# dalek-cryptography/zkp

Measured on AMD Instinct MI355X. Metric: proofs/sec + batch-verifies/sec, CMZ13 10-attr credential, 1/2/4/8 MI355X, higher is better.
Workload: dtype u32x9 (29-bit limbs, u64 accumulate)

## Files before the change

### include/zkp_mi355x.h

```cpp
#ifndef ZKP_MI355X_H
#define ZKP_MI355X_H

#include <stddef.h>
#include <stdint.h>

#ifdef __cplusplus
extern "C" {
#endif

#define ZKP_OK 0
#define ZKP_ERR_HIP (-1)
#define ZKP_ERR_ARG (-2)
#define ZKP_ERR_NO_DEVICE (-3)
#define ZKP_ERR_OOM (-4)

#define ZKP_VARTIME 0
#define ZKP_CT 1

typedef struct zkp_ctx zkp_ctx;

int zkp_ctx_create(zkp_ctx** out, int device_id);
void zkp_ctx_destroy(zkp_ctx* ctx);
int zkp_ctx_set_stream(zkp_ctx* ctx, void* hip_stream);
int zkp_ctx_synchronize(zkp_ctx* ctx);
// ... 285 lines not shown
  ZKP_K_REDUCE = 2,
  ZKP_K_SORT = 3,
  ZKP_K_BUCKET = 4,
  ZKP_K_COMBINE = 5,
  ZKP_K_TRANSCRIPT = 6,
  ZKP_K_SCALARS = 7,
  ZKP_K_TABLES = 8,
  ZKP_K_COUNT = 9
};
int zkp_ctx_last_timing(zkp_ctx* ctx, float* kernel_ms , float* total_ms);
int zkp_ctx_last_kernels(zkp_ctx* ctx, int kind, char* buf, size_t cap);
int zkp_ctx_set_profiling(zkp_ctx* ctx, int enabled);

#ifdef ZKP_BUILD_TEST_HOOKS
int zkp_debug_quad_selftest(zkp_ctx* ctx, uint32_t n, const uint8_t* pairs , uint8_t* out );
int zkp_debug_row_selftest(zkp_ctx* ctx, uint32_t n, const uint8_t* pairs , uint8_t* out );
int zkp_debug_wave_cycles(zkp_ctx* ctx, uint64_t* out, uint32_t cap);
int zkp_debug_sha512(zkp_ctx* ctx, uint64_t n, const uint8_t* msgs, const uint64_t* offsets , uint8_t* out );
int zkp_debug_last_schedule(zkp_ctx* ctx, char* buf, size_t cap);
int zkp_debug_ragged_blocks(const uint8_t* transcripts, uint32_t N, uint32_t* idx, uint32_t* blocks, uint32_t cap);
int zkp_debug_fill_workspace(zkp_ctx* ctx, size_t min_bytes, uint32_t word);
size_t zkp_debug_ws_bytes(zkp_ctx* ctx);
size_t zkp_debug_ws_count(zkp_ctx* ctx, const uint8_t* needle, size_t len);
enum { ZKP_TESTOPT_DUMMY_LAUNCHES = 1001, ZKP_TESTOPT_GENERIC_CLASSIFIER = 1002, ZKP_TESTOPT_WAVE_CYCLES = 1003, ZKP_TESTOPT_PIP_MERGE = 1004, ZKP_TESTOPT_VOUCH_REDUCED = 1005, ZKP_TESTOPT_PIP_RUN_CAP = 1006 };
#endif

#ifdef __cplusplus
}
#endif
#endif
```

### zkp_amd/csrc/hot_tables.h

```cpp
#pragma once
#include "dev_layout.h"
#include "stmt_pairs.h"

namespace zkp {

#ifndef ZKP_HOT_W
#define ZKP_HOT_W 7
#endif
constexpr int HOT_W = ZKP_HOT_W;
constexpr int HOT_WINDOWS = (257 + HOT_W - 1) / HOT_W;
constexpr int HOT_HALF = 1 << (HOT_W - 1);
constexpr int HOT_ROW = HOT_HALF + 1;
constexpr int HOT_SLOTS = 64;
constexpr int HOT_CLASSES = HOT_SLOTS + 3;
constexpr int CLASS_COMB = HOT_SLOTS, CLASS_LADDER = HOT_SLOTS + 1, CLASS_GROUP = HOT_SLOTS + 2;
constexpr uint32_t GROUP_MIN_USES = 10;
constexpr size_t HOT_SLOT_NIELS = (size_t)HOT_WINDOWS * HOT_ROW;
constexpr int HOT_ROW_CHUNKS = HOT_ROW * (int)(sizeof(dev_niels) / 16);
constexpr int HOT_COPIES = 16;
static_assert(HOT_W >= 6 && HOT_W <= 7 && HOT_W * HOT_WINDOWS >= 258, "fixed-base window shape");
constexpr bool HOT_LDS_ROWS = HOT_ROW_CHUNKS <= 256;

constexpr int HOT_FOLD_WINDOWS = 252 / HOT_W;
static_assert(HOT_FOLD_WINDOWS * HOT_W == 252 && HOT_FOLD_WINDOWS < HOT_WINDOWS, "the folded walk ends at bit 252");

constexpr uint32_t hot_pattern_word(int i, int n = HOT_WINDOWS) {
  uint32_t v = 0;
  for (int w = 0; w < n; ++w) {
    const int bit = HOT_W * w + HOT_W - 1;
    if (bit / 32 == i) v |= 1u << (bit % 32);
  }
  return v;
}
__device__ __forceinline__ void hot_recode(uint32_t e[9], const uint32_t s[8], bool fold = false) {
  constexpr uint32_t P[9] = {hot_pattern_word(0), hot_pattern_word(1), hot_pattern_word(2), hot_pattern_word(3), hot_pattern_word(4),
                             hot_pattern_word(5), hot_pattern_word(6), hot_pattern_word(7), hot_pattern_word(8)};
  constexpr uint32_t F[9] = {hot_pattern_word(0, HOT_FOLD_WINDOWS - 1), hot_pattern_word(1, HOT_FOLD_WINDOWS - 1), hot_pattern_word(2, HOT_FOLD_WINDOWS - 1),
                             hot_pattern_word(3, HOT_FOLD_WINDOWS - 1), hot_pattern_word(4, HOT_FOLD_WINDOWS - 1), hot_pattern_word(5, HOT_FOLD_WINDOWS - 1),
                             hot_pattern_word(6, HOT_FOLD_WINDOWS - 1), hot_pattern_word(7, HOT_FOLD_WINDOWS - 1), hot_pattern_word(8, HOT_FOLD_WINDOWS - 1)};
  uint64_t c = 0;
#pragma unroll
  for (int i = 0; i < 8; ++i) {
    c += (uint64_t)s[i] + (fold ? F[i] : P[i]);
    e[i] = (uint32_t)c;
    c >>= 32;
  }
  e[8] = (uint32_t)c + (fold ? F[8] : P[8]);
}
__device__ __forceinline__ void hot_next_digit(uint32_t e[9], uint32_t& mag, uint32_t& neg, bool raw = false) {
  const uint32_t d = e[0] & ((1u << HOT_W) - 1u);
#pragma unroll
  for (int i = 0; i < 8; ++i) e[i] = __builtin_amdgcn_alignbit(e[i + 1], e[i], HOT_W);
  e[8] >>= HOT_W;
  neg = raw ? 0u : (uint32_t)(d < (uint32_t)HOT_HALF);
  mag = raw ? d : neg ? (uint32_t)HOT_HALF - d : d - (uint32_t)HOT_HALF;
}

__global__ void __launch_bounds__(64, 2)
k_hot_bases(uint32_t nh, const dev_affine* __restrict__ pts, dev_ext* __restrict__ bases) {
  const uint32_t h = blockIdx.x * blockDim.x + threadIdx.x;
  if (h >= nh) return;
  ge_p3 b;
  load_affine(b, pts + h);
  ge_pin_vgpr(b);
  store_ext(bases + (size_t)h * HOT_WINDOWS, b);
#pragma unroll 1
  for (int w = 1; w < HOT_WINDOWS; ++w) {
#pragma unroll 1
    for (int k = 0; k < HOT_W - 1; ++k) ge_double<false>(b, b);
    ge_double<true>(b, b);
    store_ext(bases + (size_t)h * HOT_WINDOWS + w, b);
  }
}

__global__ void __launch_bounds__(64, 2)
k_hot_rows(uint32_t nh, const uint32_t* __restrict__ slots, const dev_ext* __restrict__ bases, dev_ext* __restrict__ mult,
           dev_niels* __restrict__ tables) {
  const uint32_t g = blockIdx.x * blockDim.x + threadIdx.x;
  if (g >= nh * HOT_WINDOWS) return;
// ... 326 lines not shown
            wd[4 * i + 0] = (wd[4 * i + 0] & ~m) | (x.x & m); wd[4 * i + 1] = (wd[4 * i + 1] & ~m) | (x.y & m);
            wd[4 * i + 2] = (wd[4 * i + 2] & ~m) | (x.z & m); wd[4 * i + 3] = (wd[4 * i + 3] & ~m) | (x.w & m);
          }
        }
      } else {
        const uint4* ent = rep + (size_t)mag * (sizeof(dev_niels) / 16) * HOT_COPIES + copy;
#pragma unroll
        for (int i = 0; i < 7; ++i) {
          const uint4 x = ent[i * HOT_COPIES];
          wd[4 * i + 0] = x.x; wd[4 * i + 1] = x.y; wd[4 * i + 2] = x.z; wd[4 * i + 3] = x.w;
        }
      }
      ge_niels q;
      fe_set(q.ypx, wd); fe_set(q.ymx, wd + 9); fe_set(q.xy2d, wd + 18);
      ge_niels_cneg(q, neg);
      if (w == 0) ge_from_niels(acc, q);
      else ge_madd(acc, acc, q);
    }
  }
}

__device__ __forceinline__ uint32_t xbar_fetch(int src_lane_x4, uint32_t v) { return (uint32_t)__builtin_amdgcn_ds_bpermute(src_lane_x4, (int)v); }

__device__ __forceinline__ void fixed_base_xbar(ge_p3& acc, uint32_t e[9], const uint4* __restrict__ rows, bool fold = false) {
  const uint32_t lane = threadIdx.x & 63u;
  constexpr int SETS = HOT_HALF / 32;
  static_assert(HOT_HALF == 32 * SETS && SETS >= 1 && SETS <= 2, "the crossbar walk holds sets of 32 entries");
  const uint4* my = rows + (size_t)(1u + (lane & 31u)) * 7u + (lane >> 5) * 4u;
  const uint32_t last = lane < 32u ? 3u : 2u;
  uint4 r[SETS][4];
#pragma unroll
  for (int s = 0; s < SETS; ++s)
#pragma unroll
    for (int q = 0; q < 4; ++q) r[s][q] = my[(size_t)s * 32 * 7 + (q < 3 ? (uint32_t)q : last)];
  const int windows = fold ? HOT_FOLD_WINDOWS : HOT_WINDOWS;
#pragma unroll 1
  for (int w = 0; w < windows; ++w) {
    uint32_t mag, neg;
    hot_next_digit(e, mag, neg, fold && w == HOT_FOLD_WINDOWS - 1);
    const uint32_t nz = (uint32_t)(mag != 0u);
    const uint32_t m1 = mag - nz;
    const int src = (int)((m1 & 31u) << 2);
    uint32_t wd[28];
#pragma unroll
    for (int s = 0; s < SETS; ++s) {
      uint32_t t[28];
#pragma unroll
      for (int q = 0; q < 4; ++q) {
        t[4 * q + 0] = xbar_fetch(src, r[s][q].x); t[4 * q + 1] = xbar_fetch(src, r[s][q].y);
        t[4 * q + 2] = xbar_fetch(src, r[s][q].z); t[4 * q + 3] = xbar_fetch(src, r[s][q].w);
      }
#pragma unroll
      for (int q = 0; q < 3; ++q) {
        t[16 + 4 * q + 0] = xbar_fetch(src + 128, r[s][q].x); t[16 + 4 * q + 1] = xbar_fetch(src + 128, r[s][q].y);
        t[16 + 4 * q + 2] = xbar_fetch(src + 128, r[s][q].z);
        if (q < 2) t[16 + 4 * q + 3] = xbar_fetch(src + 128, r[s][q].w);
      }
      if (s == 0) {
#pragma unroll
        for (int i = 0; i < 27; ++i) wd[i] = t[i];
      } else {
        const bool hi = m1 >= 32u;
#pragma unroll
        for (int i = 0; i < 27; ++i) wd[i] = hi ? t[i] : wd[i];
      }
    }
    if (w + 1 < windows) {
      const uint4* nx = my + (size_t)(w + 1) * HOT_ROW_CHUNKS;
#pragma unroll
      for (int s = 0; s < SETS; ++s)
#pragma unroll
        for (int q = 0; q < 4; ++q) r[s][q] = nx[(size_t)s * 32 * 7 + (q < 3 ? (uint32_t)q : last)];
    }
    const uint32_t m = 0u - nz;
#pragma unroll
    for (int i = 0; i < 27; ++i) wd[i] &= m;
    wd[0] |= nz ^ 1u;
    wd[9] |= nz ^ 1u;
    ge_niels q;
    fe_set(q.ypx, wd); fe_set(q.ymx, wd + 9); fe_set(q.xy2d, wd + 18);
    ge_niels_cneg(q, neg);
    if (w == 0) ge_from_niels(acc, q);
    else ge_madd(acc, acc, q);
  }
}

}
```

### zkp_amd/csrc/zkp_kernels.hip

```cpp
#include <hip/hip_runtime.h>
#include <sys/syscall.h>
#include <unistd.h>
#include <cassert>
#include <cctype>
#include <cstdio>
#include <cstring>
#include <algorithm>
#include <atomic>
#include <functional>
#include <map>
#include <memory>
#include <mutex>
#include <set>
#include <string>
#include <unordered_map>
#include <vector>
#include "../../include/zkp_mi355x.h"
#include "dev_layout.h"

using namespace zkp;

__device__ __forceinline__ uint32_t sel8(const uint32_t w[8], int j) {
  uint32_t r = w[0];
#pragma unroll
// ... 165 lines not shown
    }
    ZKP_WAVE_T1(2);
  } else if (vb < ladder_blocks + comb_blocks + group_blocks) {
    if constexpr (CT && TEETH == 16) {
      if constexpr (LOOKUP == LOOKUP_XBAR)
        comb_group_xbar((vb - ladder_blocks - comb_blocks) * XBAR_BLOCK_TERMS, n_group, list + class_start[CLASS_GROUP], scalars, pidx, slot_of, comb, partial, hot_lds, no_carry != 0);
      else
        comb_group_block((vb - ladder_blocks - comb_blocks) * 256u, n_group, list + class_start[CLASS_GROUP], scalars, pidx, slot_of, comb, partial, hot_lds, no_carry != 0);
    }
    ZKP_WAVE_T1(3);
  } else {
    const uint32_t hb = vb - ladder_blocks - comb_blocks - group_blocks;
    if (hb >= blk_start[HOT_SLOTS]) return;
    uint32_t c = 0;
    while (blk_start[c + 1] <= hb) ++c;
    const uint4* src = reinterpret_cast<const uint4*>(tables + (size_t)c * HOT_SLOT_NIELS);
    const uint32_t i = (hb - blk_start[c]) * 256 + threadIdx.x;
    const bool live = i < class_start[c + 1] - class_start[c];
    const uint32_t t = live ? list[class_start[c] + i] : 0u;
    uint32_t s[8], e[9];
    ge_p3 acc;
    ge_identity(acc);
    if constexpr (LOOKUP == LOOKUP_XBAR) {
      if (hb * 256u + (threadIdx.x & ~63u) - blk_start[c] * 256u >= class_start[c + 1] - class_start[c]) return;
#pragma unroll
      for (int q = 0; q < 8; ++q) s[q] = 0;
      if (live) load_vec<2>(s, scalars + 32 * (size_t)t);
      const bool fold = CT && no_carry;
      uint32_t flip = 0;
      if (fold) flip = sc_fold_sign(s);
      hot_recode(e, s, fold);
      fixed_base_xbar(acc, e, src, fold);
      if (fold) ge_cneg(acc, flip);
    } else {
      if (live) {
        load_vec<2>(s, scalars + 32 * (size_t)t);
        hot_recode(e, s);
      }
      fixed_base_block<LOOKUP == LOOKUP_SCAN>(acc, e, live, src, hot_lds);
    }
    if (live) store_ext(partial + t, acc);
    ZKP_WAVE_T1(4);
  }
}

struct msm_map {
  uint32_t N = 0, nc = 0;
  const uint32_t* order = nullptr;
};
__device__ __forceinline__ uint32_t msm_of_lane(const msm_map& m, uint32_t p) {
  if (!m.order) return p;
  const uint32_t q = p / m.N;
  return (p - q * m.N) * m.nc + m.order[q];
}

// ... 687 lines not shown
#pragma unroll 1
  for (int k = 0; k < shift; ++k) q_double(U, U, q);
  if (level > 0) {
    const dev_ext* ain = A_in + (size_t)w * in_stride + (size_t)m * j;
#pragma unroll 1
    for (int i = 0; i < m; ++i) {
      q_load_ext(t, ain + i, q);
      q_add(U, U, t, q);
    }
  }
  q_store_ext(A_out + (size_t)w * out_stride + j, U, q);
  if (R_out) q_store_ext(R_out + (size_t)w * out_stride + j, run, q);
}
__global__ void __launch_bounds__(256, 2)
k_pip_reduce_lvl(uint32_t n_out, uint32_t total, uint32_t in_stride, uint32_t out_stride, int level, int m, int shift,
                 const dev_ext* __restrict__ A_in, const dev_ext* __restrict__ R_in,
                 dev_ext* __restrict__ A_out, dev_ext* __restrict__ R_out) {
  const uint32_t gt = blockIdx.x * blockDim.x + threadIdx.x;
  const uint32_t g = gt >> 2;
  const int q = (int)(gt & 3u);
  if (g >= total) return;
  pip_reduce_quad(g, q, n_out, in_stride, out_stride, level, m, shift, A_in, R_in, A_out, R_out);
}

__global__ void __launch_bounds__(256)
k_pip_combine(int W1, int C, uint32_t in_stride, int level, int m, int shift, const dev_ext* __restrict__ A_in, const dev_ext* __restrict__ R_in,
              dev_ext* __restrict__ T_all, const uint32_t* __restrict__ invalid, uint8_t* __restrict__ out_point, uint32_t* __restrict__ status,
              uint32_t shared_flags ) {
  const uint32_t b = blockIdx.x;
  dev_ext* T = T_all + (size_t)b * W1;
  const uint32_t g = threadIdx.x >> 2;
  const int q = (int)(threadIdx.x & 3u);
  if (g < (uint32_t)W1) pip_reduce_quad(b * (uint32_t)W1 + g, q, 1u, in_stride, 1u, level, m, shift, A_in, R_in, T_all, nullptr);
  __syncthreads();
  __shared__ uint32_t Tl[64 * 36];
  if (g < (uint32_t)W1) {
    qpt t;
    q_load_ext(t, T + g, q);
    if (g + 1 < (uint32_t)W1) {
      qcached cc;
      q_to_cached(cc, t, q);
      t.c = cc.c;
    }
#pragma unroll
    for (int i = 0; i < 9; ++i) Tl[36 * g + 9 * q + i] = t.c.v[i];
  }
// ... 681 lines not shown
  bool batch_encode_user = false;
  int comb_teeth = 4;
  int ct_single_use_tables = -1;
  struct { bool offered = false, active = false; const tr_op* ops = nullptr; uint32_t n_ops = 0; const uint64_t* tables = nullptr; uint32_t N = 0; tr_bufs bufs{};
           uint8_t* ts = nullptr; uint32_t* saved = nullptr; uint32_t* failed = nullptr; uint32_t tail = 0;
           bool steps = false; tr_steps_dev sd; uint64_t* img = nullptr; } pending_tr;
  int debug_dummy_launches = 0;
  bool stmt_classify = true;
  int fuse_tables_transcript = -1;
  int tables_lane = -1;
  int comb_split = -1;
  int grouped_comb = -1;
  int ladder_interleave = -1;
  static constexpr uint32_t kInterleaveLadderBlocks = 256;
  bool each_straus = true;
  uint32_t each_straus_lanes = 0;
  uint32_t each_straus_wins = 0;
  int ct_lookup = 0;
#ifdef ZKP_BUILD_TEST_HOOKS
  uint64_t* wave_cycles = nullptr;
  static constexpr uint32_t kWaveCyclesCap = 1u << 20;
  enum { SCH_BATCH_ENCODE, SCH_ENC_GROUPS, SCH_OPT_PIP, SCH_PIP_C, SCH_PIP_PART, SCH_STATUS_SHARED, SCH_LAT_SPLIT, SCH_GROUPED, SCH_COMB_MIN,
         SCH_LADDER_INTERLEAVE, SCH_RIDERS, SCH_STRAUS_LANES, SCH_STRAUS_WINS, SCH_TR_LANES, SCH_TR_STEPS, SCH_FUSE_TT, SCH_TERMS_SPLIT,
         SCH_RAGGED_CLASSES, SCH_RAGGED_COMPILED, SCH_RAGGED_BASE, SCH_FUSED_PLANS, SCH_PIP_MERGE, SCH_PIP_BUCKETS, SCH_NO_CARRY, SCH_SIGN_FOLD, SCH_COUNT };
  int64_t sched[SCH_COUNT] = {-1, -1, -1, -1, -1, -1, -1, -1, -1, -1, -1, -1, -1, -1, -1, -1, -1, -1, -1, -1, -1, -1, -1, -1, -1};
  uint64_t debug_pip_run_cap = 0;
  int debug_pip_merge = 0;
  bool debug_vouch_reduced = false;
#endif
  static constexpr size_t kGroupedCombTerms = 400000;
  static constexpr size_t kSplitCombTerms = 8192;
  bool dev_overlap = false;
  bool dev_latency = false;
  bool rider_tables = true;
  bool joint_ladder = true;
  bool tr_steps = true;
  int tr_lanes = -1;
  static constexpr size_t kWideCallTerms = 250000, kWideCallProofs = 8192;
  static constexpr size_t kVeryWideCallProofs = 65536;
  uint32_t ct_comb_min(bool throughput, size_t n_terms) const {
    return ct_single_use_tables < 0 ? (throughput && n_terms >= kWideCallTerms ? 2u : 1u) : (ct_single_use_tables ? 1u : 2u);
  }
  void* ws = nullptr;
  size_t ws_bytes = 0;
  uint64_t ws_generation = 0, plans_generation = 0;
  bool profiling = false;
  hipEvent_t ev[kMaxEvents] = {};
  int ev_kind[kMaxEvents] = {};
  int n_ev = 0;
  float kernel_ms[ZKP_K_COUNT] = {};
// ... 470 lines not shown

template <int C>
uint32_t pip_tiles(uint64_t n) { return (uint32_t)((n + sort_cfg<C>::TILE - 1) / sort_cfg<C>::TILE); }

template <int C>
size_t pip_ws(uint64_t n, uint32_t K = 1) {
  using cfg = pip_cfg<C>;
  const size_t WK = (size_t)cfg::W1 * K;
  carve cv;
  cv.take((size_t)K * n * sizeof(dev_niels));
  cv.take(WK * n * 4);
  cv.take(WK * n * 4);
  cv.take(WK * cfg::B1 * 4 * 3);
  cv.take(WK * (cfg::B1 + 1) * 4);
  cv.take(WK * pip_tiles<C>(n) * cfg::B1 * 4);
  cv.take(WK * pip_vmax<C>(n) * sizeof(dev_ext));
  cv.take(WK * pip_vmax<C>(n) * 4);
  cv.take((size_t)K * 4 + 256);
  cv.take(WK * cfg::B1 * sizeof(dev_ext));
  cv.take(WK * (cfg::B + 8) * sizeof(dev_ext) * 2);
  return cv.off;
}

template <int C>
int pip_run(zkp_ctx* c, uint32_t n, const uint8_t* d_scalars, const uint8_t* d_points, uint8_t* d_out,
            uint32_t* d_status, size_t ws_reserved, uint32_t* shared_flags, const pip_seg seg = pip_seg(), int phases = 3, const pip_csr* csr = nullptr) {
  using cfg = pip_cfg<C>;
  const uint32_t K = seg.K;
  const size_t WK = (size_t)cfg::W1 * K;
  if (WK > 65535) return fail(ZKP_ERR_ARG, "too many batches in one call");
  carve cv;
  cv.off = ws_reserved;
  char* base = static_cast<char*>(c->ws);
  dev_niels* niels = reinterpret_cast<dev_niels*>(base + cv.take((size_t)K * n * sizeof(dev_niels)));
  uint32_t* digits = reinterpret_cast<uint32_t*>(base + cv.take(WK * n * 4));
  uint32_t* sorted = reinterpret_cast<uint32_t*>(base + cv.take(WK * n * 4));
  const size_t nb = WK * cfg::B1;
  if (nb * 4 > 0xffffffffull) return fail(ZKP_ERR_ARG, "too many batches in one call");
  uint32_t* hist = reinterpret_cast<uint32_t*>(base + cv.take(nb * 4 * 3));
  uint32_t* start = hist + nb;
  uint32_t* cursor = start + nb;
  uint32_t* vstart = reinterpret_cast<uint32_t*>(base + cv.take(WK * (cfg::B1 + 1) * 4));
  const uint32_t tiles = pip_tiles<C>(n);
  uint32_t* tilehist = reinterpret_cast<uint32_t*>(base + cv.take(WK * tiles * cfg::B1 * 4));
  const uint32_t L = pip_part_len(n);
  const size_t vmax = pip_vmax<C>(n);
// ... 25 lines not shown
    else hipLaunchKernelGGL((k_pip_prepare<C, 3>), dim3((n + 255) / 256, K), dim3(256), 0, c->stream, n, seg, d_scalars, d_points, niels, digits, invalid);
  }
  prof_mark(c, ZKP_K_DECODE);
  hipLaunchKernelGGL(k_pip_tile_hist<C>, dim3(tiles, (unsigned)WK), dim3(sort_cfg<C>::THREADS), 0, c->stream, n, digits, tilehist);
  hipLaunchKernelGGL(k_pip_tile_total, grid1(nb, 256), dim3(256), 0, c->stream, cfg::B1, tiles, (uint32_t)nb, tilehist, hist);
  hipLaunchKernelGGL(k_pip_scan, dim3((unsigned)WK), dim3(256), 0, c->stream, cfg::B1, L, hist, start, cursor, vstart);
  hipLaunchKernelGGL(k_pip_tile_base, grid1(nb, 256), dim3(256), 0, c->stream, cfg::B1, tiles, (uint32_t)nb, start, tilehist);
  hipLaunchKernelGGL(k_pip_tile_scatter<C>, dim3(tiles, (unsigned)WK), dim3(sort_cfg<C>::THREADS), 0, c->stream, n, digits, tilehist, sorted);
  prof_mark(c, ZKP_K_SORT);
  hipLaunchKernelGGL(k_pip_vmap, grid1(nb, 256), dim3(256), 0, c->stream, cfg::B1, (uint32_t)nb, (uint32_t)vmax, vstart, vmap);
  hipLaunchKernelGGL(k_pip_bucket_part, dim3((unsigned)((vmax + 255) / 256), (unsigned)WK), dim3(256), 0, c->stream, n, (uint32_t)cfg::W1, cfg::B1, L, (uint32_t)vmax,
                     start, hist, vstart, vmap, sorted, niels, parts);
  constexpr size_t MERGE_LANE_MIN_BUCKETS = (size_t)1 << 19;
#ifdef ZKP_BUILD_TEST_HOOKS
  const bool lane_merge = c->debug_pip_merge ? c->debug_pip_merge == 2 : nb >= MERGE_LANE_MIN_BUCKETS;
#else
  const bool lane_merge = nb >= MERGE_LANE_MIN_BUCKETS;
#endif
  ZKP_SCHED(c, PIP_MERGE, lane_merge ? 1 : 0);
  ZKP_SCHED(c, PIP_BUCKETS, nb);
  if (lane_merge) hipLaunchKernelGGL(k_pip_bucket_merge<true>, grid1(nb, 256), dim3(256), 0, c->stream, cfg::B1, (uint32_t)nb, (uint32_t)vmax, vstart, parts, buckets);
  else hipLaunchKernelGGL(k_pip_bucket_merge<false>, grid1(nb * 4, 256), dim3(256), 0, c->stream, cfg::B1, (uint32_t)nb, (uint32_t)vmax, vstart, parts, buckets);
  prof_mark(c, ZKP_K_BUCKET);
  const dev_ext* Ain = nullptr;
  const dev_ext* Rin = buckets;
  uint32_t in_stride = cfg::B1, n_in = cfg::B;
  size_t lvl_off = 0;
  int level = 0;
  int shift = 0;
  static_assert(cfg::W1 <= 64, "k_pip_combine runs the last tree level with one quad per window in one 256-lane block");
  while (n_in > 1) {
    int lg = 0;
    while ((1u << lg) < n_in) ++lg;
    const int mbits = (level == 0 && lg % 3) ? lg % 3 : 3;
    const uint32_t m = 1u << mbits, n_out = n_in >> mbits;
    dev_ext* Aout = lvlA + lvl_off;
    dev_ext* Rout = lvlR + lvl_off;
    const uint32_t total = (uint32_t)WK * n_out;
    if (n_out == 1) {
      hipLaunchKernelGGL(k_pip_combine, dim3(K), dim3(256), 0, c->stream, cfg::W1, C, in_stride, level, (int)m, shift, Ain, Rin, Aout, invalid, d_out, d_status, shared_flags ? 1u : 0u);
      break;
    }
    hipLaunchKernelGGL(k_pip_reduce_lvl, grid1((size_t)total * 4, 256), dim3(256), 0, c->stream, n_out, total, in_stride, n_out, level, (int)m, shift,
                       Ain, Rin, Aout, Rout);
    Ain = Aout;
    Rin = Rout;
    in_stride = n_out;
    n_in = n_out;
    lvl_off += total;
    shift += mbits;
    ++level;
  }
  prof_mark(c, ZKP_K_COMBINE);
  HIP_TRY(hipGetLastError());
  return ZKP_OK;
}

int pick_c(uint64_t n) {
  if (n < (1u << 12)) return 7;
  if (n < (1u << 13)) return 10;
  if (n < (1u << 21)) return 11;
  return 16;
}
constexpr uint64_t kSmallOptional = 192;
inline size_t pip_ws_for(int cbits, uint64_t n, uint32_t K = 1) {
  switch (cbits) {
    case 7: return pip_ws<7>(n, K);
// ... 741 lines not shown
  free_ragged_progs(c);
  if (c->side_stream) hipStreamDestroy(c->side_stream);
  if (c->ev_fork) hipEventDestroy(c->ev_fork);
  if (c->ev_join) hipEventDestroy(c->ev_join);
  for (auto& e : c->ev) if (e) hipEventDestroy(e);
  if (c->own_stream) hipStreamDestroy(c->own_stream);
  delete c;
}

int zkp_ctx_set_stream(zkp_ctx* c, void* s) {
  if (!c) return fail(ZKP_ERR_ARG, "ctx is NULL");
  c->stream = s ? static_cast<hipStream_t>(s) : c->own_stream;
  return ZKP_OK;
}
int zkp_ctx_set_option(zkp_ctx* c, int option, uint64_t value) {
  if (!c) return fail(ZKP_ERR_ARG, "ctx is NULL");
  switch (option) {
    case ZKP_OPT_BATCH_ENCODE_MIN: c->batch_encode_min = value; c->batch_encode_user = true; return ZKP_OK;
    case ZKP_OPT_CT_SINGLE_USE_TABLES: c->ct_single_use_tables = value == ~0ull ? -1 : (value ? 1 : 0); return ZKP_OK;
    case ZKP_OPT_DEV_OVERLAP: c->dev_overlap = value != 0 && value != ~0ull; c->dev_latency = value == 2; return ZKP_OK;
#ifdef ZKP_BUILD_TEST_HOOKS
    case ZKP_TESTOPT_GENERIC_CLASSIFIER: c->stmt_classify = value == 0; return ZKP_OK;
    case ZKP_TESTOPT_PIP_MERGE: c->debug_pip_merge = value <= 2 ? (int)value : 0; return ZKP_OK;
    case ZKP_TESTOPT_VOUCH_REDUCED: c->debug_vouch_reduced = value != 0; return ZKP_OK;
    case ZKP_TESTOPT_PIP_RUN_CAP: c->debug_pip_run_cap = value; return ZKP_OK;
    case ZKP_TESTOPT_DUMMY_LAUNCHES: c->debug_dummy_launches = (int)std::min<uint64_t>(value, 1000); return ZKP_OK;
    case ZKP_TESTOPT_WAVE_CYCLES: {
      HIP_TRY(hipSetDevice(c->device));
      HIP_TRY(hipStreamSynchronize(c->stream));
      uint64_t* p = nullptr;
      uint32_t cap = 0;
      if (value) {
        if (!c->wave_cycles) HIP_TRY(hipMalloc(&c->wave_cycles, sizeof(uint64_t) * zkp_ctx::kWaveCyclesCap));
        HIP_TRY(hipMemset(c->wave_cycles, 0, sizeof(uint64_t) * zkp_ctx::kWaveCyclesCap));
        p = c->wave_cycles;
        cap = zkp_ctx::kWaveCyclesCap;
      }
      HIP_TRY(hipMemcpyToSymbol(HIP_SYMBOL(g_wave_cycles), &p, sizeof(p)));
      HIP_TRY(hipMemcpyToSymbol(HIP_SYMBOL(g_wave_cycles_cap), &cap, sizeof(cap)));
      return ZKP_OK;
    }
#endif
    case ZKP_OPT_FUSE_TABLES_TRANSCRIPT: c->fuse_tables_transcript = value == ~0ull ? -1 : (value ? 1 : 0); return ZKP_OK;
    case ZKP_OPT_TABLES_LANE: c->tables_lane = value == ~0ull ? -1 : (value ? 1 : 0); return ZKP_OK;
    case ZKP_OPT_GROUPED_COMB: c->grouped_comb = value == ~0ull ? -1 : (value ? 1 : 0); return ZKP_OK;
    case ZKP_OPT_JOINT_LADDER: c->joint_ladder = value != 0; c->rider_tables = value != 2; return ZKP_OK;
// ... 1144 lines not shown
int zkp_transcripts_append_points(zkp_ctx* c, uint32_t N, uint8_t* ts, const char* kind, const char* var_label, const uint8_t* points, int validate,
                                  uint8_t* status) {
  strobe_label k, v;
  bool done;
  int rc = append_points_check(c, N, kind, var_label, k, v, &done);
  if (rc || done) return rc;
  if (!ts || !points || (validate && !status)) return fail(ZKP_ERR_ARG, "NULL pointer");
  if (!strobe_positions_ok(ts, N)) return fail(ZKP_ERR_ARG, "a transcript's position byte is 166 or more");
  HIP_TRY(hipSetDevice(c->device));
  staging st(c);
  const size_t o_ts = st.inout(ts, ts, 208 * (size_t)N);
  const size_t o_pts = st.in(points, 32 * (size_t)N);
  const size_t o_st = st.out_opt(status, (size_t)N);
  rc = st.begin();
  if (rc) return rc;
  return st.end(launch_strobe_append_points(c, N, st.at<uint8_t>(o_ts), k, v, st.at<uint8_t>(o_pts), validate ? 1u : 0u, st.at<uint8_t>(o_st)));
}

#ifdef ZKP_BUILD_TEST_HOOKS
int zkp_debug_last_schedule(zkp_ctx* c, char* buf, size_t cap) {
  if (!c || !buf || !cap) return fail(ZKP_ERR_ARG, "bad argument");
  static const char* const names[zkp_ctx::SCH_COUNT] = {"batch_encode", "enc_groups", "opt_pip", "pip_c", "pip_part", "status_shared", "lat_split", "grouped", "comb_min",
                                                        "ladder_interleave", "riders", "straus_lanes", "straus_wins", "tr_lanes", "tr_steps", "fuse_tt", "terms_split",
                                                        "ragged_classes", "ragged_compiled", "ragged_base", "fused_plans", "pip_merge", "pip_buckets", "no_carry", "sign_fold"};
  std::string s;
  for (int i = 0; i < zkp_ctx::SCH_COUNT; ++i)
    if (c->sched[i] >= 0) s += (s.empty() ? "" : " ") + std::string(names[i]) + "=" + std::to_string(c->sched[i]);
  const size_t n = std::min(s.size(), cap - 1);
  memcpy(buf, s.data(), n);
  buf[n] = 0;
  return (int)s.size();
}

int zkp_debug_sha512(zkp_ctx* c, uint64_t n, const uint8_t* msgs, const uint64_t* offsets, uint8_t* out) {
  return hash_from_bytes_host(c, n, msgs, offsets, out, HASH_DIGEST);
}
#endif

#ifdef ZKP_BUILD_TEST_HOOKS
int zkp_debug_quad_selftest(zkp_ctx* c, uint32_t n, const uint8_t* pairs, uint8_t* out) {
  if (!c || !pairs || !out) return fail(ZKP_ERR_ARG, "NULL pointer");
  if (n == 0) return ZKP_OK;
  HIP_TRY(hipSetDevice(c->device));
  staging st(c);
  const size_t o_in = st.in(pairs, (size_t)n * 64);
  const size_t o_out = st.out(out, (size_t)n * 128);
  const int rc = st.upload();
// ... 98 lines not shown
```

### zkp_amd/engine.py

```python
from __future__ import annotations

import ctypes
import os
from typing import Optional, Sequence, Tuple

import numpy as np

from . import cabi

_HERE = os.path.dirname(os.path.abspath(__file__))
LIB_PATH = os.path.join(_HERE, "libzkp_mi355x.so")
TESTHOOKS_LIB_PATH = os.path.join(_HERE, "libzkp_mi355x_testhooks.so")
ZKP_TESTOPT_DUMMY_LAUNCHES, ZKP_TESTOPT_GENERIC_CLASSIFIER, ZKP_TESTOPT_WAVE_CYCLES, ZKP_TESTOPT_PIP_MERGE, ZKP_TESTOPT_VOUCH_REDUCED = 1001, 1002, 1003, 1004, 1005
ZKP_TESTOPT_PIP_RUN_CAP = 1006
ZKP_OPT_CT_LOOKUP, ZKP_OPT_EACH_STRAUS, ZKP_OPT_LADDER_INTERLEAVE = 9, 10, 11
ZKP_OPT_CT_MASKED_SCANS = ZKP_OPT_CT_LOOKUP
ZKP_CT_LOOKUP_XBAR, ZKP_CT_LOOKUP_SCAN, ZKP_CT_LOOKUP_LDS = 0, 1, 2
ZKP_OPT_WS_LIMIT_BYTES, ZKP_OPT_JOB_DEFER_D2H, ZKP_OPT_SYNC_SCHEDULE, ZKP_OPT_TRANSCRIPT_STEPS, ZKP_OPT_COMB_SPLIT, ZKP_OPT_JOINT_LADDER = 12, 13, 14, 15, 16, 17

ZKP_VARTIME = 0
ZKP_CT = 1
ZKP_RNG_SCALARS = 0
ZKP_RNG_BYTES = 1
ZKP_PT_ADD, ZKP_PT_SUB = 0, 1
ZKP_SC_SUM, ZKP_SC_PRODUCT, ZKP_SC_DOT = 0, 1, 2
ZKP_SCAN_INCLUSIVE, ZKP_SCAN_EXCLUSIVE = 0, 1
ZKP_DLOG_FOUND, ZKP_DLOG_INVALID, ZKP_DLOG_NOT_FOUND = 0, 1, 2
ZKP_DLOG_SLOTS, ZKP_DLOG_SIGNED = 8, 1
ZKP_OPT_BATCH_ENCODE_MIN = 1
(ZKP_OPT_COMB_TEETH, ZKP_OPT_CT_SINGLE_USE_TABLES, ZKP_OPT_TRANSCRIPT_LANES, ZKP_OPT_DEV_OVERLAP, ZKP_OPT_GROUPED_COMB, ZKP_OPT_TABLES_LANE,
 ZKP_OPT_FUSE_TABLES_TRANSCRIPT) = 2, 3, 4, 5, 6, 7, 8
K_NAMES = ("decode", "terms", "reduce", "sort", "bucket", "combine", "transcript", "scalars", "tables")

EXPORTS = tuple(cabi.signatures("zkp_mi355x.h"))
TEST_HOOK_EXPORTS = tuple(cabi.signatures("zkp_mi355x.h", test_hooks=True))


# ... 866 lines not shown
```

Baseline: 4.608 million.

## Widen fixed-base window to 8 bits, stage rows in LDS, add per-lane PIP tree reduce

Raises the default fixed-base window width from 7 to 8 bits, which cuts the number of windows and point additions per scalar multiplication. To serve the wider rows it adds an LDS double-buffered staging path: loader waves prefetch the next window's table row into LDS while walker waves do the crossbar lookup, so every wave reads rows from LDS instead of global memory. Separately it adds a one-thread-per-output PIP tree reduction kernel, used for large bucket counts, and exposes a test hook to force either tree path. The trade-offs are larger tables and LDS use, plus a barrier per window that keeps inactive waves in the block instead of letting them exit early.

```diff
diff --git a/include/zkp_mi355x.h b/include/zkp_mi355x.h
--- a/include/zkp_mi355x.h
+++ b/include/zkp_mi355x.h
@@ -331,7 +331,7 @@
 int zkp_debug_fill_workspace(zkp_ctx* ctx, size_t min_bytes, uint32_t word);
 size_t zkp_debug_ws_bytes(zkp_ctx* ctx);
 size_t zkp_debug_ws_count(zkp_ctx* ctx, const uint8_t* needle, size_t len);
-enum { ZKP_TESTOPT_DUMMY_LAUNCHES = 1001, ZKP_TESTOPT_GENERIC_CLASSIFIER = 1002, ZKP_TESTOPT_WAVE_CYCLES = 1003, ZKP_TESTOPT_PIP_MERGE = 1004, ZKP_TESTOPT_VOUCH_REDUCED = 1005, ZKP_TESTOPT_PIP_RUN_CAP = 1006 };
+enum { ZKP_TESTOPT_DUMMY_LAUNCHES = 1001, ZKP_TESTOPT_GENERIC_CLASSIFIER = 1002, ZKP_TESTOPT_WAVE_CYCLES = 1003, ZKP_TESTOPT_PIP_MERGE = 1004, ZKP_TESTOPT_VOUCH_REDUCED = 1005, ZKP_TESTOPT_PIP_RUN_CAP = 1006, ZKP_TESTOPT_PIP_TREE = 1007 };
 #endif
 
 #ifdef __cplusplus
diff --git a/zkp_amd/csrc/hot_recode.h b/zkp_amd/csrc/hot_recode.h
--- /dev/null
+++ b/zkp_amd/csrc/hot_recode.h
@@ -0,0 +1,60 @@
+#pragma once
+#include <stdint.h>
+#include "fe25519.h"
+
+namespace zkp {
+
+#ifndef ZKP_HOT_W
+#define ZKP_HOT_W 8
+#endif
+constexpr int HOT_W = ZKP_HOT_W;
+constexpr int HOT_WINDOWS = (257 + HOT_W - 1) / HOT_W;
+constexpr int HOT_HALF = 1 << (HOT_W - 1);
+
+constexpr int HOT_FOLD_WINDOWS = (252 + HOT_W - 1) / HOT_W;
+constexpr int HOT_FOLD_TOP_BIT = HOT_W * (HOT_FOLD_WINDOWS - 1);
+constexpr int HOT_FOLD_LAST_MAX = 1 << (251 - HOT_FOLD_TOP_BIT);
+static_assert(HOT_FOLD_TOP_BIT < 252 && HOT_FOLD_WINDOWS * HOT_W >= 252 && HOT_FOLD_WINDOWS < HOT_WINDOWS, "the folded walk covers bits 0 .. 251 and saves a window");
+static_assert(HOT_FOLD_TOP_BIT > 125, "the excess of (l - 1) / 2 over 2^251, below 2^124, and the offsets lie below the last window");
+static_assert(HOT_FOLD_LAST_MAX <= HOT_HALF, "the last window of a folded walk, read without the offset, names a table entry");
+
+constexpr uint32_t hot_pattern_word(int i, int n = HOT_WINDOWS) {
+  uint32_t v = 0;
+  for (int w = 0; w < n; ++w) {
+    const int bit = HOT_W * w + HOT_W - 1;
+    if (bit / 32 == i) v |= 1u << (bit % 32);
+  }
+  return v;
+}
+ZKP_HD void hot_recode(uint32_t e[9], const uint32_t s[8], bool fold = false) {
+  constexpr uint32_t P[9] = {hot_pattern_word(0), hot_pattern_word(1), hot_pattern_word(2), hot_pattern_word(3), hot_pattern_word(4),
+                             hot_pattern_word(5), hot_pattern_word(6), hot_pattern_word(7), hot_pattern_word(8)};
+  constexpr uint32_t F[9] = {hot_pattern_word(0, HOT_FOLD_WINDOWS - 1), hot_pattern_word(1, HOT_FOLD_WINDOWS - 1), hot_pattern_word(2, HOT_FOLD_WINDOWS - 1),
+                             hot_pattern_word(3, HOT_FOLD_WINDOWS - 1), hot_pattern_word(4, HOT_FOLD_WINDOWS - 1), hot_pattern_word(5, HOT_FOLD_WINDOWS - 1),
+                             hot_pattern_word(6, HOT_FOLD_WINDOWS - 1), hot_pattern_word(7, HOT_FOLD_WINDOWS - 1), hot_pattern_word(8, HOT_FOLD_WINDOWS - 1)};
+  uint64_t c = 0;
+#pragma unroll
+  for (int i = 0; i < 8; ++i) {
+    c += (uint64_t)s[i] + (fold ? F[i] : P[i]);
+    e[i] = (uint32_t)c;
+    c >>= 32;
+  }
+  e[8] = (uint32_t)c + (fold ? F[8] : P[8]);
+}
+ZKP_HD uint32_t hot_funnel(uint32_t hi, uint32_t lo) {
+#if defined(__HIP_DEVICE_COMPILE__)
+  return __builtin_amdgcn_alignbit(hi, lo, HOT_W);
+#else
+  return (uint32_t)((((uint64_t)hi << 32) | lo) >> HOT_W);
+#endif
+}
+ZKP_HD void hot_next_digit(uint32_t e[9], uint32_t& mag, uint32_t& neg, bool raw = false) {
+  const uint32_t d = e[0] & ((1u << HOT_W) - 1u);
+#pragma unroll
+  for (int i = 0; i < 8; ++i) e[i] = hot_funnel(e[i + 1], e[i]);
+  e[8] >>= HOT_W;
+  neg = raw ? 0u : (uint32_t)(d < (uint32_t)HOT_HALF);
+  mag = raw ? d : neg ? (uint32_t)HOT_HALF - d : d - (uint32_t)HOT_HALF;
+}
+
+}
diff --git a/zkp_amd/csrc/hot_tables.h b/zkp_amd/csrc/hot_tables.h
--- a/zkp_amd/csrc/hot_tables.h
+++ b/zkp_amd/csrc/hot_tables.h
@@ -1,15 +1,10 @@
 #pragma once
 #include "dev_layout.h"
+#include "hot_recode.h"
 #include "stmt_pairs.h"
 
 namespace zkp {
 
-#ifndef ZKP_HOT_W
-#define ZKP_HOT_W 7
-#endif
-constexpr int HOT_W = ZKP_HOT_W;
-constexpr int HOT_WINDOWS = (257 + HOT_W - 1) / HOT_W;
-constexpr int HOT_HALF = 1 << (HOT_W - 1);
 constexpr int HOT_ROW = HOT_HALF + 1;
 constexpr int HOT_SLOTS = 64;
 constexpr int HOT_CLASSES = HOT_SLOTS + 3;
@@ -18,43 +13,8 @@
 constexpr size_t HOT_SLOT_NIELS = (size_t)HOT_WINDOWS * HOT_ROW;
 constexpr int HOT_ROW_CHUNKS = HOT_ROW * (int)(sizeof(dev_niels) / 16);
 constexpr int HOT_COPIES = 16;
-static_assert(HOT_W >= 6 && HOT_W <= 7 && HOT_W * HOT_WINDOWS >= 258, "fixed-base window shape");
+static_assert(HOT_W >= 6 && HOT_W <= 8 && HOT_W * HOT_WINDOWS >= 258, "fixed-base window shape");
 constexpr bool HOT_LDS_ROWS = HOT_ROW_CHUNKS <= 256;
-
-constexpr int HOT_FOLD_WINDOWS = 252 / HOT_W;
-static_assert(HOT_FOLD_WINDOWS * HOT_W == 252 && HOT_FOLD_WINDOWS < HOT_WINDOWS, "the folded walk ends at bit 252");
-
-constexpr uint32_t hot_pattern_word(int i, int n = HOT_WINDOWS) {
-  uint32_t v = 0;
-  for (int w = 0; w < n; ++w) {
-    const int bit = HOT_W * w + HOT_W - 1;
-    if (bit / 32 == i) v |= 1u << (bit % 32);
-  }
-  return v;
-}
-__device__ __forceinline__ void hot_recode(uint32_t e[9], const uint32_t s[8], bool fold = false) {
-  constexpr uint32_t P[9] = {hot_pattern_word(0), hot_pattern_word(1), hot_pattern_word(2), hot_pattern_word(3), hot_pattern_word(4),
-                             hot_pattern_word(5), hot_pattern_word(6), hot_pattern_word(7), hot_pattern_word(8)};
-  constexpr uint32_t F[9] = {hot_pattern_word(0, HOT_FOLD_WINDOWS - 1), hot_pattern_word(1, HOT_FOLD_WINDOWS - 1), hot_pattern_word(2, HOT_FOLD_WINDOWS - 1),
-                             hot_pattern_word(3, HOT_FOLD_WINDOWS - 1), hot_pattern_word(4, HOT_FOLD_WINDOWS - 1), hot_pattern_word(5, HOT_FOLD_WINDOWS - 1),
-                             hot_pattern_word(6, HOT_FOLD_WINDOWS - 1), hot_pattern_word(7, HOT_FOLD_WINDOWS - 1), hot_pattern_word(8, HOT_FOLD_WINDOWS - 1)};
-  uint64_t c = 0;
-#pragma unroll
-  for (int i = 0; i < 8; ++i) {
-    c += (uint64_t)s[i] + (fold ? F[i] : P[i]);
-    e[i] = (uint32_t)c;
-    c >>= 32;
-  }
-  e[8] = (uint32_t)c + (fold ? F[8] : P[8]);
-}
-__device__ __forceinline__ void hot_next_digit(uint32_t e[9], uint32_t& mag, uint32_t& neg, bool raw = false) {
-  const uint32_t d = e[0] & ((1u << HOT_W) - 1u);
-#pragma unroll
-  for (int i = 0; i < 8; ++i) e[i] = __builtin_amdgcn_alignbit(e[i + 1], e[i], HOT_W);
-  e[8] >>= HOT_W;
-  neg = raw ? 0u : (uint32_t)(d < (uint32_t)HOT_HALF);
-  mag = raw ? d : neg ? (uint32_t)HOT_HALF - d : d - (uint32_t)HOT_HALF;
-}
 
 __global__ void __launch_bounds__(64, 2)
 k_hot_bases(uint32_t nh, const dev_affine* __restrict__ pts, dev_ext* __restrict__ bases) {
@@ -427,15 +387,52 @@
 
 __device__ __forceinline__ uint32_t xbar_fetch(int src_lane_x4, uint32_t v) { return (uint32_t)__builtin_amdgcn_ds_bpermute(src_lane_x4, (int)v); }
 
+__device__ __forceinline__ void xbar_take_set(uint32_t wd[28], const uint4 r[4], int src, uint32_t m1, int S) {
+  uint32_t t[28];
+#pragma unroll
+  for (int q = 0; q < 4; ++q) {
+    t[4 * q + 0] = xbar_fetch(src, r[q].x); t[4 * q + 1] = xbar_fetch(src, r[q].y);
+    t[4 * q + 2] = xbar_fetch(src, r[q].z); t[4 * q + 3] = xbar_fetch(src, r[q].w);
+  }
+#pragma unroll
+  for (int q = 0; q < 3; ++q) {
+    t[16 + 4 * q + 0] = xbar_fetch(src + 128, r[q].x); t[16 + 4 * q + 1] = xbar_fetch(src + 128, r[q].y);
+    t[16 + 4 * q + 2] = xbar_fetch(src + 128, r[q].z);
+    if (q < 2) t[16 + 4 * q + 3] = xbar_fetch(src + 128, r[q].w);
+  }
+  if (S == 0) {
+#pragma unroll
+    for (int i = 0; i < 27; ++i) wd[i] = t[i];
+  } else {
+    const bool mine = (m1 >> 5) == (uint32_t)S;
+#pragma unroll
+    for (int i = 0; i < 27; ++i) wd[i] = mine ? t[i] : wd[i];
+  }
+}
+__device__ __forceinline__ void xbar_add_entry(ge_p3& acc, uint32_t wd[28], uint32_t nz, uint32_t neg, bool first) {
+  const uint32_t m = 0u - nz;
+#pragma unroll
+  for (int i = 0; i < 27; ++i) wd[i] &= m;
+  wd[0] |= nz ^ 1u;
+  wd[9] |= nz ^ 1u;
+  ge_niels q;
+  fe_set(q.ypx, wd); fe_set(q.ymx, wd + 9); fe_set(q.xy2d, wd + 18);
+  ge_niels_cneg(q, neg);
+  if (first) ge_from_niels(acc, q);
+  else ge_madd(acc, acc, q);
+}
+
+constexpr int XBAR_SETS = HOT_HALF / 32;
+static_assert(HOT_HALF == 32 * XBAR_SETS && (XBAR_SETS == 1 || XBAR_SETS == 2 || XBAR_SETS == 4), "the crossbar walks hold sets of 32 entries");
+
 __device__ __forceinline__ void fixed_base_xbar(ge_p3& acc, uint32_t e[9], const uint4* __restrict__ rows, bool fold = false) {
   const uint32_t lane = threadIdx.x & 63u;
-  constexpr int SETS = HOT_HALF / 32;
-  static_assert(HOT_HALF == 32 * SETS && SETS >= 1 && SETS <= 2, "the crossbar walk holds sets of 32 entries");
+  constexpr int SETS = XBAR_SETS, HELD = SETS < 2 ? SETS : 2, PASSES = SETS / HELD;
   const uint4* my = rows + (size_t)(1u + (lane & 31u)) * 7u + (lane >> 5) * 4u;
   const uint32_t last = lane < 32u ? 3u : 2u;
-  uint4 r[SETS][4];
-#pragma unroll
-  for (int s = 0; s < SETS; ++s)
+  uint4 r[HELD][4];
+#pragma unroll
+  for (int s = 0; s < HELD; ++s)
 #pragma unroll
     for (int q = 0; q < 4; ++q) r[s][q] = my[(size_t)s * 32 * 7 + (q < 3 ? (uint32_t)q : last)];
   const int windows = fold ? HOT_FOLD_WINDOWS : HOT_WINDOWS;
@@ -448,46 +445,76 @@
     const int src = (int)((m1 & 31u) << 2);
     uint32_t wd[28];
 #pragma unroll
-    for (int s = 0; s < SETS; ++s) {
-      uint32_t t[28];
-#pragma unroll
-      for (int q = 0; q < 4; ++q) {
-        t[4 * q + 0] = xbar_fetch(src, r[s][q].x); t[4 * q + 1] = xbar_fetch(src, r[s][q].y);
-        t[4 * q + 2] = xbar_fetch(src, r[s][q].z); t[4 * q + 3] = xbar_fetch(src, r[s][q].w);
-      }
-#pragma unroll
-      for (int q = 0; q < 3; ++q) {
-        t[16 + 4 * q + 0] = xbar_fetch(src + 128, r[s][q].x); t[16 + 4 * q + 1] = xbar_fetch(src + 128, r[s][q].y);
-        t[16 + 4 * q + 2] = xbar_fetch(src + 128, r[s][q].z);
-        if (q < 2) t[16 + 4 * q + 3] = xbar_fetch(src + 128, r[s][q].w);
-      }
-      if (s == 0) {
-#pragma unroll
-        for (int i = 0; i < 27; ++i) wd[i] = t[i];
-      } else {
-        const bool hi = m1 >= 32u;
-#pragma unroll
-        for (int i = 0; i < 27; ++i) wd[i] = hi ? t[i] : wd[i];
-      }
+    for (int p = 0; p < PASSES; ++p) {
+      if (p > 0) {
+        const uint4* cur = my + (size_t)w * HOT_ROW_CHUNKS + (size_t)p * HELD * 32 * 7;
+#pragma unroll
+        for (int s = 0; s < HELD; ++s)
+#pragma unroll
+          for (int q = 0; q < 4; ++q) r[s][q] = cur[(size_t)s * 32 * 7 + (q < 3 ? (uint32_t)q : last)];
+      }
+#pragma unroll
+      for (int s = 0; s < HELD; ++s) xbar_take_set(wd, r[s], src, m1, p * HELD + s);
     }
     if (w + 1 < windows) {
       const uint4* nx = my + (size_t)(w + 1) * HOT_ROW_CHUNKS;
 #pragma unroll
-      for (int s = 0; s < SETS; ++s)
+      for (int s = 0; s < HELD; ++s)
 #pragma unroll
         for (int q = 0; q < 4; ++q) r[s][q] = nx[(size_t)s * 32 * 7 + (q < 3 ? (uint32_t)q : last)];
     }
-    const uint32_t m = 0u - nz;
-#pragma unroll
-    for (int i = 0; i < 27; ++i) wd[i] &= m;
-    wd[0] |= nz ^ 1u;
-    wd[9] |= nz ^ 1u;
-    ge_niels q;
-    fe_set(q.ypx, wd); fe_set(q.ymx, wd + 9); fe_set(q.xy2d, wd + 18);
-    ge_niels_cneg(q, neg);
-    if (w == 0) ge_from_niels(acc, q);
-    else ge_madd(acc, acc, q);
-  }
-}
-
-}
+    xbar_add_entry(acc, wd, nz, neg, w == 0);
+  }
+}
+
+#ifndef ZKP_HOT_STAGE_ROWS
+#define ZKP_HOT_STAGE_ROWS 1
+#endif
+constexpr int HOT_STAGE_UINT4 = XBAR_SETS * 4 * 64;
+__device__ __forceinline__ void fixed_base_staged(ge_p3& acc, uint32_t e[9], const uint4* __restrict__ rows, bool fold, bool walk, uint4* stage) {
+  const uint32_t lane = threadIdx.x & 63u, wave = threadIdx.x >> 6;
+  constexpr int SETS = XBAR_SETS;
+  const bool loader = wave < (uint32_t)SETS;
+  const uint4* my = rows + (size_t)(1u + 32u * (loader ? wave : 0u) + (lane & 31u)) * 7u + (lane >> 5) * 4u;
+  const uint32_t last = lane < 32u ? 3u : 2u;
+  uint4* put = stage + wave * 256u + lane;
+  const uint4* get = stage + lane;
+  uint4 pf0 = make_uint4(0, 0, 0, 0), pf1 = pf0, pf2 = pf0, pf3 = pf0;
+  if (loader) {
+    pf0 = my[0]; pf1 = my[1]; pf2 = my[2]; pf3 = my[last];
+    put[0] = pf0; put[64] = pf1; put[128] = pf2; put[192] = pf3;
+  }
+  const int windows = fold ? HOT_FOLD_WINDOWS : HOT_WINDOWS;
+#pragma unroll 1
+  for (int w = 0; w < windows; ++w) {
+    lds_barrier();
+    const bool more = loader && w + 1 < windows;
+    if (more) {
+      const uint4* nx = my + (size_t)(w + 1) * HOT_ROW_CHUNKS;
+      pf0 = nx[0]; pf1 = nx[1]; pf2 = nx[2]; pf3 = nx[last];
+    }
+    if (walk) {
+      uint32_t mag, neg;
+      hot_next_digit(e, mag, neg, fold && w == HOT_FOLD_WINDOWS - 1);
+      const uint32_t nz = (uint32_t)(mag != 0u);
+      const uint32_t m1 = mag - nz;
+      const int src = (int)((m1 & 31u) << 2);
+      const uint4* row = get + (w & 1) * HOT_STAGE_UINT4;
+      uint32_t wd[28];
+#pragma unroll
+      for (int s = 0; s < SETS; ++s) {
+        uint4 r[4];
+#pragma unroll
+        for (int q = 0; q < 4; ++q) r[q] = row[(4 * s + q) * 64];
+        xbar_take_set(wd, r, src, m1, s);
+      }
+      xbar_add_entry(acc, wd, nz, neg, w == 0);
+    }
+    if (more) {
+      uint4* nxt = put + ((w + 1) & 1) * HOT_STAGE_UINT4;
+      nxt[0] = pf0; nxt[64] = pf1; nxt[128] = pf2; nxt[192] = pf3;
+    }
+  }
+}
+
+}
diff --git a/zkp_amd/csrc/zkp_kernels.hip b/zkp_amd/csrc/zkp_kernels.hip
--- a/zkp_amd/csrc/zkp_kernels.hip
+++ b/zkp_amd/csrc/zkp_kernels.hip
@@ -211,7 +211,7 @@
     ge_p3 acc;
     ge_identity(acc);
     if constexpr (LOOKUP == LOOKUP_XBAR) {
-      if (hb * 256u + (threadIdx.x & ~63u) - blk_start[c] * 256u >= class_start[c + 1] - class_start[c]) return;
+      const bool walk = hb * 256u + (threadIdx.x & ~63u) - blk_start[c] * 256u < class_start[c + 1] - class_start[c];
 #pragma unroll
       for (int q = 0; q < 8; ++q) s[q] = 0;
       if (live) load_vec<2>(s, scalars + 32 * (size_t)t);
@@ -219,7 +219,13 @@
       uint32_t flip = 0;
       if (fold) flip = sc_fold_sign(s);
       hot_recode(e, s, fold);
+#if ZKP_HOT_STAGE_ROWS
+      static_assert(2 * HOT_STAGE_UINT4 <= terms_lds_uint4<LOOKUP>(), "two staged rows fit the block's LDS");
+      fixed_base_staged(acc, e, src, fold, walk, hot_lds);
+#else
+      if (!walk) return;
       fixed_base_xbar(acc, e, src, fold);
+#endif
       if (fold) ge_cneg(acc, flip);
     } else {
       if (live) {
@@ -953,6 +959,45 @@
   if (g >= total) return;
   pip_reduce_quad(g, q, n_out, in_stride, out_stride, level, m, shift, A_in, R_in, A_out, R_out);
 }
+__global__ void __launch_bounds__(256, 2)
+k_pip_reduce_lvl_lane(uint32_t n_out, uint32_t total, uint32_t in_stride, int level, int m, int shift,
+                      const dev_ext* __restrict__ A_in, const dev_ext* __restrict__ R_in,
+                      dev_ext* __restrict__ A_out, dev_ext* __restrict__ R_out) {
+  const uint32_t g = blockIdx.x * blockDim.x + threadIdx.x;
+  if (g >= total) return;
+  const uint32_t w = g / n_out, j = g - w * n_out;
+  const dev_ext* rin = R_in + (size_t)w * in_stride + (size_t)m * j;
+  int i = (level == 0 && j == n_out - 1) ? m : m - 1;
+  ge_p3 run, U, t;
+  load_ext(run, rin + i);
+  U = run;
+  load_ext(t, rin + i - 1);
+#pragma unroll 1
+  for (--i; i >= 1; --i) {
+    ge_cached c;
+    ge_to_cached(c, t);
+    load_ext(t, rin + i - 1);
+    ge_add_cached(run, run, c);
+    ge_add_p3(U, U, run);
+  }
+  ge_add_p3(run, run, t);
+#pragma unroll 1
+  for (int k = 1; k < shift; ++k) ge_double<false>(U, U);
+  if (shift > 0) ge_double<true>(U, U);
+  if (level > 0) {
+    const dev_ext* ain = A_in + (size_t)w * in_stride + (size_t)m * j;
+    load_ext(t, ain);
+#pragma unroll 1
+    for (int a = 0; a < m; ++a) {
+      ge_cached c;
+      ge_to_cached(c, t);
+      if (a + 1 < m) load_ext(t, ain + a + 1);
+      ge_add_cached(U, U, c);
+    }
+  }
+  store_ext(A_out + (size_t)w * n_out + j, U);
+  store_ext(R_out + (size_t)w * n_out + j, run);
+}
 
 __global__ void __launch_bounds__(256)
 k_pip_combine(int W1, int C, uint32_t in_stride, int level, int m, int shift, const dev_ext* __restrict__ A_in, const dev_ext* __restrict__ R_in,
@@ -1680,10 +1725,11 @@
   static constexpr uint32_t kWaveCyclesCap = 1u << 20;
   enum { SCH_BATCH_ENCODE, SCH_ENC_GROUPS, SCH_OPT_PIP, SCH_PIP_C, SCH_PIP_PART, SCH_STATUS_SHARED, SCH_LAT_SPLIT, SCH_GROUPED, SCH_COMB_MIN,
          SCH_LADDER_INTERLEAVE, SCH_RIDERS, SCH_STRAUS_LANES, SCH_STRAUS_WINS, SCH_TR_LANES, SCH_TR_STEPS, SCH_FUSE_TT, SCH_TERMS_SPLIT,
-         SCH_RAGGED_CLASSES, SCH_RAGGED_COMPILED, SCH_RAGGED_BASE, SCH_FUSED_PLANS, SCH_PIP_MERGE, SCH_PIP_BUCKETS, SCH_NO_CARRY, SCH_SIGN_FOLD, SCH_COUNT };
-  int64_t sched[SCH_COUNT] = {-1, -1, -1, -1, -1, -1, -1, -1, -1, -1, -1, -1, -1, -1, -1, -1, -1, -1, -1, -1, -1, -1, -1, -1, -1};
+         SCH_RAGGED_CLASSES, SCH_RAGGED_COMPILED, SCH_RAGGED_BASE, SCH_FUSED_PLANS, SCH_PIP_MERGE, SCH_PIP_BUCKETS, SCH_NO_CARRY, SCH_SIGN_FOLD, SCH_PIP_TREE, SCH_COUNT };
+  int64_t sched[SCH_COUNT] = {-1, -1, -1, -1, -1, -1, -1, -1, -1, -1, -1, -1, -1, -1, -1, -1, -1, -1, -1, -1, -1, -1, -1, -1, -1, -1};
   uint64_t debug_pip_run_cap = 0;
   int debug_pip_merge = 0;
+  int debug_pip_tree = 0;
   bool debug_vouch_reduced = false;
 #endif
   static constexpr size_t kGroupedCombTerms = 400000;
@@ -2200,6 +2246,9 @@
   return cv.off;
 }
 
+#ifndef ZKP_PIP_TREE_LANE_MIN_OUTPUTS
+#define ZKP_PIP_TREE_LANE_MIN_OUTPUTS (1u << 16)
+#endif
 template <int C>
 int pip_run(zkp_ctx* c, uint32_t n, const uint8_t* d_scalars, const uint8_t* d_points, uint8_t* d_out,
             uint32_t* d_status, size_t ws_reserved, uint32_t* shared_flags, const pip_seg seg = pip_seg(), int phases = 3, const pip_csr* csr = nullptr) {
@@ -2271,6 +2320,14 @@
   if (lane_merge) hipLaunchKernelGGL(k_pip_bucket_merge<true>, grid1(nb, 256), dim3(256), 0, c->stream, cfg::B1, (uint32_t)nb, (uint32_t)vmax, vstart, parts, buckets);
   else hipLaunchKernelGGL(k_pip_bucket_merge<false>, grid1(nb * 4, 256), dim3(256), 0, c->stream, cfg::B1, (uint32_t)nb, (uint32_t)vmax, vstart, parts, buckets);
   prof_mark(c, ZKP_K_BUCKET);
+#ifdef ZKP_BUILD_TEST_HOOKS
+  const bool lane_tree = c->debug_pip_tree ? c->debug_pip_tree == 2 : nb >= MERGE_LANE_MIN_BUCKETS;
+  const uint32_t TREE_LANE_MIN_OUTPUTS = c->debug_pip_tree == 2 ? 0u : (uint32_t)ZKP_PIP_TREE_LANE_MIN_OUTPUTS;
+#else
+  const bool lane_tree = nb >= MERGE_LANE_MIN_BUCKETS;
+  constexpr uint32_t TREE_LANE_MIN_OUTPUTS = ZKP_PIP_TREE_LANE_MIN_OUTPUTS;
+#endif
+  ZKP_SCHED(c, PIP_TREE, 0);
   const dev_ext* Ain = nullptr;
   const dev_ext* Rin = buckets;
   uint32_t in_stride = cfg::B1, n_in = cfg::B;
@@ -2290,8 +2347,13 @@
       hipLaunchKernelGGL(k_pip_combine, dim3(K), dim3(256), 0, c->stream, cfg::W1, C, in_stride, level, (int)m, shift, Ain, Rin, Aout, invalid, d_out, d_status, shared_flags ? 1u : 0u);
       break;
     }
-    hipLaunchKernelGGL(k_pip_reduce_lvl, grid1((size_t)total * 4, 256), dim3(256), 0, c->stream, n_out, total, in_stride, n_out, level, (int)m, shift,
-                       Ain, Rin, Aout, Rout);
+    if (lane_tree && total >= TREE_LANE_MIN_OUTPUTS) {
+      ZKP_SCHED(c, PIP_TREE, level + 1);
+      hipLaunchKernelGGL(k_pip_reduce_lvl_lane, grid1(total, 256), dim3(256), 0, c->stream, n_out, total, in_stride, level, (int)m, shift, Ain, Rin, Aout, Rout);
+    } else {
+      hipLaunchKernelGGL(k_pip_reduce_lvl, grid1((size_t)total * 4, 256), dim3(256), 0, c->stream, n_out, total, in_stride, n_out, level, (int)m, shift,
+                         Ain, Rin, Aout, Rout);
+    }
     Ain = Aout;
     Rin = Rout;
     in_stride = n_out;
@@ -3079,6 +3141,7 @@
 #ifdef ZKP_BUILD_TEST_HOOKS
     case ZKP_TESTOPT_GENERIC_CLASSIFIER: c->stmt_classify = value == 0; return ZKP_OK;
     case ZKP_TESTOPT_PIP_MERGE: c->debug_pip_merge = value <= 2 ? (int)value : 0; return ZKP_OK;
+    case ZKP_TESTOPT_PIP_TREE: c->debug_pip_tree = value <= 2 ? (int)value : 0; return ZKP_OK;
     case ZKP_TESTOPT_VOUCH_REDUCED: c->debug_vouch_reduced = value != 0; return ZKP_OK;
     case ZKP_TESTOPT_PIP_RUN_CAP: c->debug_pip_run_cap = value; return ZKP_OK;
     case ZKP_TESTOPT_DUMMY_LAUNCHES: c->debug_dummy_launches = (int)std::min<uint64_t>(value, 1000); return ZKP_OK;
@@ -4269,7 +4332,7 @@
   if (!c || !buf || !cap) return fail(ZKP_ERR_ARG, "bad argument");
   static const char* const names[zkp_ctx::SCH_COUNT] = {"batch_encode", "enc_groups", "opt_pip", "pip_c", "pip_part", "status_shared", "lat_split", "grouped", "comb_min",
                                                         "ladder_interleave", "riders", "straus_lanes", "straus_wins", "tr_lanes", "tr_steps", "fuse_tt", "terms_split",
-                                                        "ragged_classes", "ragged_compiled", "ragged_base", "fused_plans", "pip_merge", "pip_buckets", "no_carry", "sign_fold"};
+                                                        "ragged_classes", "ragged_compiled", "ragged_base", "fused_plans", "pip_merge", "pip_buckets", "no_carry", "sign_fold", "pip_tree"};
   std::string s;
   for (int i = 0; i < zkp_ctx::SCH_COUNT; ++i)
     if (c->sched[i] >= 0) s += (s.empty() ? "" : " ") + std::string(names[i]) + "=" + std::to_string(c->sched[i]);
diff --git a/zkp_amd/engine.py b/zkp_amd/engine.py
--- a/zkp_amd/engine.py
+++ b/zkp_amd/engine.py
@@ -13,6 +13,7 @@
 TESTHOOKS_LIB_PATH = os.path.join(_HERE, "libzkp_mi355x_testhooks.so")
 ZKP_TESTOPT_DUMMY_LAUNCHES, ZKP_TESTOPT_GENERIC_CLASSIFIER, ZKP_TESTOPT_WAVE_CYCLES, ZKP_TESTOPT_PIP_MERGE, ZKP_TESTOPT_VOUCH_REDUCED = 1001, 1002, 1003, 1004, 1005
 ZKP_TESTOPT_PIP_RUN_CAP = 1006
+ZKP_TESTOPT_PIP_TREE = 1007
 ZKP_OPT_CT_LOOKUP, ZKP_OPT_EACH_STRAUS, ZKP_OPT_LADDER_INTERLEAVE = 9, 10, 11
 ZKP_OPT_CT_MASKED_SCANS = ZKP_OPT_CT_LOOKUP
 ZKP_CT_LOOKUP_XBAR, ZKP_CT_LOOKUP_SCAN, ZKP_CT_LOOKUP_LDS = 0, 1, 2
```

Result: no change. 4.584 million (-0.5%).
